# razorheadfx/aether_primitives

Hardware: AMD Instinct MI355X
Metric: GSamples/s cf32 (FFT-2048 + 64-tap FIR chain) (higher is better)
Workload: dtype f32; 1 GPU; C3: 64-tap FIR via overlap-save (FFT-2048) on 16 Mi cf32 samples per step (one fused kernel launch), device-resident, rotating over 6 stream pairs = 1536 MiB; fft_len=2048, ntaps=64, hop=1984, queues_per_gpu=2, parallelism=1 independent stream(s), one per GPU, no collective

## Files before the change

### aether_primitives_amd/csrc/aeth_fft_core.h

```cpp
#pragma once

#include <hip/hip_runtime.h>

#ifndef AETH_LDS_DB_LIMIT
#define AETH_LDS_DB_LIMIT (36 * 1024)
#endif

namespace aeth {
namespace fftk {

typedef float cf __attribute__((ext_vector_type(2)));

__device__ __forceinline__ cf mk(float a, float b) { cf r = {a, b}; return r; }

__device__ __forceinline__ cf cadd(cf a, cf b)
{
    cf d; asm("v_pk_add_f32 %0, %1, %2" : "=v"(d) : "v"(a), "v"(b)); return d;
}
__device__ __forceinline__ cf csub(cf a, cf b)
{
    cf d; asm("v_pk_add_f32 %0, %1, %2 neg_lo:[0,1] neg_hi:[0,1]" : "=v"(d) : "v"(a), "v"(b)); return d;
}
__device__ __forceinline__ cf cadd_mjb(cf a, cf b)
{
    cf d; asm("v_pk_add_f32 %0, %1, %2 op_sel:[0,1] op_sel_hi:[1,0] neg_lo:[0,0] neg_hi:[0,1]" : "=v"(d) : "v"(a), "v"(b));
    return d;
}
__device__ __forceinline__ cf cadd_pjb(cf a, cf b)
{
    cf d; asm("v_pk_add_f32 %0, %1, %2 op_sel:[0,1] op_sel_hi:[1,0] neg_lo:[0,1] neg_hi:[0,0]" : "=v"(d) : "v"(a), "v"(b));
    return d;
}
template <int S> __device__ __forceinline__ cf cadd_rot(cf a, cf b) { return S < 0 ? cadd_mjb(a, b) : cadd_pjb(a, b); }
template <int S> __device__ __forceinline__ cf csub_rot(cf a, cf b) { return S < 0 ? cadd_pjb(a, b) : cadd_mjb(a, b); }

// ... 147 lines not shown
        dft4_inplace<S, false>(o0, o1, o2, o3);
        u[0] = cadd(e0, o0);        u[4] = csub(e0, o0);
        bfly_w8<S, 1>(e1, o1, hh, u[1], u[5]);
        u[2] = cadd_rot<S>(e2, o2); u[6] = csub_rot<S>(e2, o2);
        bfly_w8<S, 3>(e3, o3, hh, u[3], u[7]);
    }
};

template <int S> struct Bfly<16, S> {
    static __device__ __forceinline__ void run(cf (&u)[16])
    {
        const cf hh = mk(kSqrtHalf, kSqrtHalf);
        const cf w1 = mk(kCosPi8, -kSinPi8), w3 = mk(kSinPi8, -kCosPi8), w9 = mk(-kCosPi8, kSinPi8);
        dft4_inplace<S, false>(u[0], u[4], u[8],  u[12]);
        dft4_inplace<S, false>(u[1], u[5], u[9],  u[13]);
        dft4_inplace<S, false>(u[2], u[6], u[10], u[14]);
        dft4_inplace<S, false>(u[3], u[7], u[11], u[15]);
        cf c0[4] = {u[0], u[1], u[2], u[3]};
        cf c1[4] = {u[4], ctw_k<S>(u[5], w1), cmul_w8<S, 1>(u[6], hh), ctw_k<S>(u[7], w3)};
        cf c2[4] = {u[8], cmul_w8<S, 1>(u[9], hh), u[10], cmul_w8<S, 3>(u[11], hh)};
        cf c3[4] = {u[12], ctw_k<S>(u[13], w3), cmul_w8<S, 3>(u[14], hh), ctw_k<S>(u[15], w9)};
        dft4_inplace<S, false>(c0[0], c0[1], c0[2], c0[3]);
        dft4_inplace<S, false>(c1[0], c1[1], c1[2], c1[3]);
        dft4_inplace<S, true>(c2[0], c2[1], c2[2], c2[3]);
        dft4_inplace<S, false>(c3[0], c3[1], c3[2], c3[3]);
#pragma unroll
        for (int kq = 0; kq < 4; kq++) {
            u[0 + 4 * kq] = c0[kq];
            u[1 + 4 * kq] = c1[kq];
            u[2 + 4 * kq] = c2[kq];
            u[3 + 4 * kq] = c3[kq];
        }
    }
};

constexpr double kPiD = 3.14159265358979323846264338327950288;
constexpr double c_sin_taylor(double x)
{
    double term = x, sum = x;
    for (int k = 1; k < 14; k++) { term *= -x * x / ((2 * k) * (2 * k + 1)); sum += term; }
    return sum;
}
constexpr double c_sin(double x)
{
    while (x > kPiD) x -= 2 * kPiD;
    while (x < -kPiD) x += 2 * kPiD;
    if (x > kPiD / 2) x = kPiD - x;
    if (x < -kPiD / 2) x = -kPiD - x;
    return c_sin_taylor(x);
}
constexpr double c_cos(double x) { return c_sin(x + kPiD / 2); }

template <int S> struct Bfly<3, S> {
    static __device__ __forceinline__ void run(cf (&u)[3])
    {
        constexpr float s60 = (float)c_sin(kPiD / 3);
        const cf t1 = cadd(u[1], u[2]), t2 = csub(u[1], u[2]);
        const cf y0 = cadd(u[0], t1);
        const cf h = cadd(y0, cscale_k(t1, mk(-1.5f, -1.5f)));
        const cf jt = cscale_k(t2, mk(s60, s60));
        u[0] = y0;
        u[1] = cadd_rot<S>(h, jt);
        u[2] = csub_rot<S>(h, jt);
    }
};

// ... 227 lines not shown
        }
    }
}

template <class C>
__device__ __forceinline__ void load_twiddles_lane(cf (&tw)[C::TW], const cf *__restrict__ twL, int tid)
{
    if constexpr (C::NPASS > 1) lane_tw_pass<C, 1>(tw, twL, tid, false);
    if constexpr (C::NPASS > 2) lane_tw_pass<C, 2>(tw, twL, tid, false);
    if constexpr (C::NPASS > 3) lane_tw_pass<C, 3>(tw, twL, tid, false);
}

template <class C>
__global__ void build_lane_twiddles(const cf *__restrict__ twN, cf *__restrict__ twL)
{
    const int tid = threadIdx.x;
    if (tid >= C::T) return;
    cf tw[C::TW];
    load_twiddles<C>(tw, twN, tid);
    if constexpr (C::NPASS > 1) lane_tw_pass<C, 1>(tw, twL, tid, true);
    if constexpr (C::NPASS > 2) lane_tw_pass<C, 2>(tw, twL, tid, true);
    if constexpr (C::NPASS > 3) lane_tw_pass<C, 3>(tw, twL, tid, true);
}

template <int XP> __device__ __forceinline__ void wg_barrier()
{
    if constexpr (XP & 16) {
        asm volatile("s_waitcnt lgkmcnt(0)" ::: "memory");
        __builtin_amdgcn_s_barrier();
        asm volatile("" ::: "memory");
    } else __syncthreads();
}

template <class C, int PASS, int S, int PAR, int XP = 0>
__device__ __forceinline__ void run_pass(cf (&w)[C::P], const cf (&tw)[C::TW], cf *__restrict__ lds, int tid)
{
    constexpr int R = C::radix(PASS), B = C::P / R, p = C::pbefore(PASS);
    constexpr bool last = (PASS == C::NPASS - 1);
    constexpr bool NOLDS = (XP & 4) != 0;
    cf *img = lds;
    if constexpr (!last && !NOLDS) {
        if constexpr (C::DB) img = lds + (((PAR + PASS) & 1) ? C::LDS_ELEMS : 0);
        else if constexpr (XP & 2) __builtin_amdgcn_fence(__ATOMIC_RELEASE, "workgroup");
        else wg_barrier<XP>();
    }
#pragma unroll
    for (int b = 0; b < B; b++) {
        cf u[R];
#pragma unroll
        for (int r = 0; r < R; r++) u[r] = w[b + r * B];
        if constexpr (p > 1) {
#pragma unroll
            for (int r = 1; r < R; r++) u[r] = ctw<S>(u[r], tw[C::twoff(PASS) + b * (R - 1) + (r - 1)]);
        }
        Bfly<R, S>::run(u);
        if constexpr (last || NOLDS) {
#pragma unroll
            for (int r = 0; r < R; r++) w[b + r * B] = u[r];
        } else {
            const int i = tid + b * C::T;
            const int k = i % p;
            const int j = (i - k) * R + k;
#pragma unroll
            for (int r = 0; r < R; r++) img[pidx<XP>(j + r * p)] = u[r];
        }
    }
    if constexpr (!last && !NOLDS) {
        if constexpr (XP & 1) __builtin_amdgcn_s_setprio(1);
        if constexpr (XP & 2) __builtin_amdgcn_fence(__ATOMIC_RELEASE, "workgroup");
        else wg_barrier<XP>();
#pragma unroll
        for (int m = 0; m < C::P; m++) w[m] = img[pidx<XP>(tid + m * C::T)];
        if constexpr (XP & 1) __builtin_amdgcn_s_setprio(0);
    }
}

template <class C, int S, int PAR = 0, int XP = 0>
__device__ __forceinline__ void fft_in_regs(cf (&w)[C::P], const cf (&tw)[C::TW], cf *__restrict__ lds, int tid)
{
    run_pass<C, 0, S, PAR, XP>(w, tw, lds, tid);
    if constexpr (C::NPASS > 1) run_pass<C, 1, S, PAR, XP>(w, tw, lds, tid);
    if constexpr (C::NPASS > 2) run_pass<C, 2, S, PAR, XP>(w, tw, lds, tid);
    if constexpr (C::NPASS > 3) run_pass<C, 3, S, PAR, XP>(w, tw, lds, tid);
}
template <class C> constexpr int fft_next_par(int par) { return (par + C::NPASS - 1) & 1; }

template <int N> struct CfgFor;
template <> struct CfgFor<2>    { using type = Cfg<2, 2, 2>; };
template <> struct CfgFor<4>    { using type = Cfg<4, 4, 4>; };
template <> struct CfgFor<8>    { using type = Cfg<8, 8, 8>; };
template <> struct CfgFor<16>   { using type = Cfg<16, 16, 16>; };
template <> struct CfgFor<32>   { using type = Cfg<32, 8, 8, 4>; };
template <> struct CfgFor<64>   { using type = Cfg<64, 8, 8, 8>; };
template <> struct CfgFor<128>  { using type = Cfg<128, 16, 16, 8>; };
template <> struct CfgFor<256>  { using type = Cfg<256, 16, 16, 16>; };
template <> struct CfgFor<512>  { using type = Cfg<512, 8, 8, 8, 8>; };
template <> struct CfgFor<1024> { using type = Cfg<1024, 16, 16, 16, 4>; };
template <> struct CfgFor<2048> { using type = Cfg<2048, 16, 16, 16, 8>; };
template <> struct CfgFor<4096> { using type = Cfg<4096, 16, 16, 16, 16>; };
template <> struct CfgFor<8192> { using type = Cfg<8192, 16, 16, 16, 8, 4>; };

#define AETH_POW2_SWITCH(len, BODY, DEFAULT)                                            \
    switch (len) {                                                                     \
    case 2: BODY(2); case 4: BODY(4); case 8: BODY(8); case 16: BODY(16);              \
    case 32: BODY(32); case 64: BODY(64); case 128: BODY(128); case 256: BODY(256);    \
    case 512: BODY(512); case 1024: BODY(1024); case 2048: BODY(2048);                 \
    case 4096: BODY(4096);                                                             \
    default: DEFAULT;                                                                  \
    }

#define AETH_POW2_SWITCH_XL(len, BODY, DEFAULT)                                         \
    switch (len) {                                                                     \
    case 2: BODY(2); case 4: BODY(4); case 8: BODY(8); case 16: BODY(16);              \
    case 32: BODY(32); case 64: BODY(64); case 128: BODY(128); case 256: BODY(256);    \
    case 512: BODY(512); case 1024: BODY(1024); case 2048: BODY(2048);                 \
    case 4096: BODY(4096); case 8192: BODY(8192);                                      \
// ... 6 lines not shown
```

### aether_primitives_amd/csrc/aeth_fir.hip

```cpp
#include "aeth_internal.h"
#include "aeth_fft_core.h"
#include "aeth_fft_plan.h"
#include "aeth_fir_kernel.h"
#include "aeth_host.h"

#include <cstdlib>
#include <memory>
#include <new>
#include <type_traits>
#include <vector>

using namespace aeth::fftk;


using namespace aeth::firk;

namespace {

constexpr bool fused_store_len(size_t n) { return 1024 <= n && n <= 4096; }

template <class C, bool SCALED, int MINW, bool CHIRP, int VAR, bool ONLY_NT = false>
int fmi_go(bool nt, int grid, hipStream_t stream, const FmiArgs &b)
{
    if (ONLY_NT || nt) hipLaunchKernelGGL((fmi_kernel<C, SCALED, MINW, true, CHIRP, VAR>), dim3(grid), dim3(C::WG), 0, stream, b);
// ... 34 lines not shown
                constexpr int DV = VAR | V_DEMOD | decltype(dmv)::value;
                if constexpr (kLab8) {
                    if (lab8_four) return fmi_go<C, SCALED, 4, false, DV, true>(nt, grid, stream, b);
                }
                return fmi_go<C, SCALED, 1, false, DV>(nt, grid, stream, b);
            };
            if (b.bps == 1) return demod(std::integral_constant<int, V_DM_BPSK>());
            if (b.demod_sep) return demod(std::integral_constant<int, 0>());
            return demod(std::integral_constant<int, V_DM_QGEN>());
        }
    }
    if constexpr (kStoreVariants && !SCALED) {
        if (b.dec.d > 1) {
            constexpr int DV = (VAR & ~V_XOR) | V_DECIM;
            return fmi_go<C, false, 2, false, DV>(nt, grid, stream, b);
        }
    }
    if constexpr (!(kStoreVariants && !SCALED)) {
        if (b.levels || b.parts)
            return aeth::set_error(AETH_E_UNSUPPORTED, "fused FFT*H*IFFT: no level-storing / peak-finding build of length %d", C::N);
    }
    if constexpr (kStoreVariants && !SCALED) {
        if (b.levels || b.parts) {
            const bool cnt = aeth::streams_past_cache((size_t)a.n * (b.levels ? 12 : 8));
            if (b.parts) return fmi_go<C, false, 2, false, VAR | V_PEAK>(cnt, grid, stream, b);
            if (b.level_kind == AETH_LEVEL_NORM) return fmi_go<C, false, 2, false, VAR | V_LEVEL>(cnt, grid, stream, b);
            if (b.level_kind == AETH_LEVEL_DB) return fmi_go<C, false, 2, false, VAR | V_LEVEL | V_LV_DB>(cnt, grid, stream, b);
            return fmi_go<C, false, 2, false, VAR | V_LEVEL | V_LV_POWER_DB>(cnt, grid, stream, b);
        }
    }
    if constexpr (C::F == 1 && !SCALED && C::NPASS == 3) {
        const int sp = aeth::tuning_int("AETH_FIR_SPREAD", -1);
        const bool chained = ctx->overlap && !ctx->stream_shared && ctx->last_chained;
        if (nt && (sp < 0 ? !chained : sp != 0)) return fmi_go<C, false, 1, false, VAR | V_SPREAD, true>(nt, grid, stream, b);
    }
    return fmi_go<C, SCALED, 1, false, VAR>(nt, grid, stream, b);
}

int dispatch_fmi(aeth_ctx *ctx, size_t fft_len, const FmiArgs &a, hipStream_t stream = nullptr)
{
    if (!stream) stream = aeth::ctx_stream(ctx);
    aeth::DeviceGuard dev_guard(ctx->device);
    const bool scaled = a.chirp != nullptr || !(a.s_fwd == 1.0f && a.s_bwd == 1.0f);
#if AETH_LAB
    if (fft_len == 2048 && a.bits && !a.chirp && aeth::lab_int("AETH_DEMOD_P8", 0)) {
        FmiArgs b8 = a;
        b8.twL = nullptr;
        using C8 = Cfg<2048, 8, 8, 8, 8, 4>;
        return scaled ? launch_fmi<C8, true>(ctx, b8, stream) : launch_fmi<C8, false>(ctx, b8, stream);
    }
#endif
#define AETH_BODY(NN)                                                            \
    return scaled ? launch_fmi<typename CfgFor<NN>::type, true>(ctx, a, stream)  \
                  : launch_fmi<typename CfgFor<NN>::type, false>(ctx, a, stream)
    AETH_POW2_SWITCH(fft_len, AETH_BODY, return aeth::set_error(AETH_E_UNSUPPORTED, "fused FFT*H*IFFT: length %zu", fft_len))
#undef AETH_BODY
}

bool is_pow2(size_t n) { return n && (n & (n - 1)) == 0; }

bool touch_bytes(const void *a, size_t na, const void *b, size_t nb)
{
    if (!a || !b || !na || !nb) return false;
    const uintptr_t a0 = (uintptr_t)a, a1 = a0 + na, b0 = (uintptr_t)b, b1 = b0 + nb;
    return a0 < b1 && b0 < a1;
}
bool touch(const aeth_cf32 *a, size_t na, const aeth_cf32 *b, size_t nb)
// ... 397 lines not shown
```

### aether_primitives_amd/csrc/aeth_fir_kernel.h

```cpp
#pragma once

#include "aeth_internal.h"
#include "aeth_fft_core.h"
#include "aeth_levels.h"

namespace aeth {
namespace firk {

using namespace aeth::fftk;

struct __attribute__((aligned(16))) PeakPart {
    double q;
    unsigned e;
    unsigned nnan;
};
static_assert(sizeof(PeakPart) == 16, "one 16-byte store per wave and block");
constexpr unsigned kPeakNone = 0x7fffffffu;

struct FmiArgs {
    const cf *in;
    cf *out;
    const cf *hist;
    const cf *Hf;
    const cf *twN;
// ... 2 lines not shown
    long long nblocks;
    int hop, ov, nhist;
    float s_fwd, s_bwd;
    const cf *chirp = nullptr;
    int frame_n = 0;
    int conj = 0;
    aeth::FastDiv dec = {1, 0, 0, 0};
    long long n_out = 0;
    unsigned char *bits = nullptr;
    cf tab[4] = {};
    int bps = 0, demod_compat = 0;
    int demod_sep = 0;
    float *levels = nullptr;
    int level_kind = 0;
    PeakPart *parts = nullptr;
};

enum : int {
    V_PEEL  = 1,
    V_TOUCH = 2,
    V_PRIO  = 4,
    V_TOUCH3 = 8,
    V_DECIM = 512,
    V_UNROLL2 = 4096,
    V_XOR = 2048,
    V_XCD = 8192,
    V_SPREAD = 16384,
    V_DEMOD = 1024,
    V_DM_BPSK = 1 << 16, V_DM_QGEN = 1 << 17,
    V_LEVEL = 1 << 19,
    V_LV_DB = 1 << 20, V_LV_POWER_DB = 1 << 21,
    V_PEAK = 1 << 22,
    V_DMA = 1 << 18,
    V_NOLOAD = 16,
    V_NOSTORE = 32,
    V_CENSUS = 256,
    V_NOLDS = 128,
    V_NOBAR = 64,
};

constexpr int V_PRODUCT_MASK = V_PRIO | V_XOR | V_SPREAD | V_DECIM | V_DEMOD | V_DM_BPSK | V_DM_QGEN | V_LEVEL | V_LV_DB |
                               V_LV_POWER_DB | V_PEAK;
#ifndef AETH_FIR_LAB
#define AETH_FIR_LAB 0
#endif

#ifndef AETH_FIR_LOAD_AUX
#define AETH_FIR_LOAD_AUX 2
#endif
#ifndef AETH_FIR_STORE_AUX
#define AETH_FIR_STORE_AUX 18
#endif

typedef unsigned int u32x2 __attribute__((ext_vector_type(2)));


__device__ __forceinline__ cf as_cf(u32x2 v) { return __builtin_bit_cast(cf, v); }
__device__ __forceinline__ u32x2 as_u32x2(cf v) { return __builtin_bit_cast(u32x2, v); }

template <class C, bool NT>
__device__ __forceinline__ void load_window(cf (&x)[C::P], const FmiArgs &a, long long blk, int tid)
{
    const long long win0 = blk * a.hop - a.ov;
    if (blk >= a.nblocks) {
#pragma unroll
        for (int m = 0; m < C::P; m++) x[m] = mk(0.f, 0.f);
        return;
    }
    if constexpr (C::F == 1) {
        if (win0 >= 0) {
            long long left = a.n - win0;
            int bytes = (int)(left < a.frame_n ? left : a.frame_n) * 8;
            auto rs = __builtin_amdgcn_make_buffer_rsrc(const_cast<cf *>(a.in + win0), 0, bytes, 0x00020000);
#pragma unroll
            for (int m = 0; m < C::P; m++)
// ... 3 lines not shown
    }
    if constexpr (C::F > 1) {
        const long long first = (blk - (long long)(threadIdx.x / C::T)) * a.hop - a.ov;
        const long long last_end = first + (long long)(C::F - 1) * a.hop + C::N;
        if (a.frame_n == C::N && first >= 0 && last_end <= a.n && blk - (long long)(threadIdx.x / C::T) + C::F <= a.nblocks) {
#pragma unroll
            for (int m = 0; m < C::P; m++) {
                const cf v = a.in[win0 + tid + m * C::T];
                x[m] = (tid + m * C::T >= a.ov - a.nhist) ? v : mk(0.f, 0.f);
            }
            return;
        }
        if (a.frame_n < C::N && a.ov == 0 && blk - (long long)(threadIdx.x / C::T) + C::F <= a.nblocks) {
#pragma unroll
            for (int m = 0; m < C::P; m++) {
                const int e = tid + m * C::T;
                x[m] = e < a.frame_n ? a.in[win0 + e] : mk(0.f, 0.f);
            }
            return;
        }
    }
#pragma unroll
    for (int m = 0; m < C::P; m++) {
        const long long gi = win0 + tid + m * C::T;
        cf v = mk(0.f, 0.f);
        if (tid + m * C::T >= a.ov - a.nhist && tid + m * C::T < a.frame_n) {
            if (gi >= 0) { if (gi < a.n) v = a.in[gi]; }
            else if (a.hist && gi >= -(long long)a.nhist) v = a.hist[a.nhist + gi];
        }
        x[m] = v;
    }
}

template <class C, bool NT>
__device__ __forceinline__ void load_window_srd(cf (&x)[C::P], const FmiArgs &a, long long blk, int tid)
{
    const bool active = blk < a.nblocks;
    const long long win0 = active ? blk * a.hop - a.ov : 0;
    long long left = a.n - win0;
    const int bytes = active ? (int)(left < a.frame_n ? left : a.frame_n) * 8 : 0;
    auto rs = __builtin_amdgcn_make_buffer_rsrc(const_cast<cf *>(a.in + win0), 0, bytes, 0x00020000);
#pragma unroll
    for (int m = 0; m < C::P; m++)
        x[m] = as_cf(__builtin_amdgcn_raw_buffer_load_b64(rs, (tid + m * C::T) * 8, 0, NT ? AETH_FIR_LOAD_AUX : 0));
}

template <class C, bool NT, int M0, int M1>
__device__ __forceinline__ void load_window_srd_part(cf (&x)[C::P], const FmiArgs &a, long long blk, int tid)
{
    const bool active = blk < a.nblocks;
    const long long win0 = active ? blk * a.hop - a.ov : 0;
    long long left = a.n - win0;
    const int bytes = active ? (int)(left < a.frame_n ? left : a.frame_n) * 8 : 0;
    auto rs = __builtin_amdgcn_make_buffer_rsrc(const_cast<cf *>(a.in + win0), 0, bytes, 0x00020000);
#pragma unroll
    for (int m = M0; m < M1; m++)
        x[m] = as_cf(__builtin_amdgcn_raw_buffer_load_b64(rs, (tid + m * C::T) * 8, 0, NT ? AETH_FIR_LOAD_AUX : 0));
    __builtin_amdgcn_sched_barrier(0);
}

typedef __attribute__((address_space(3))) void *lds_vptr_t;
template <bool NT>
__device__ __forceinline__ void dma_piece(__amdgpu_buffer_rsrc_t rs, cf *dst, int voff, int soff)
{
#if __HIP_DEVICE_COMPILE__
    __builtin_amdgcn_raw_ptr_buffer_load_lds(rs, (lds_vptr_t)dst, 16, voff, soff, 0, NT ? AETH_FIR_LOAD_AUX : 0);
#endif
}
template <class C, bool NT, int J0, int J1>
__device__ __forceinline__ void dma_window_part(cf *land, const FmiArgs &a, long long blk, int tid)
{
    static_assert(C::T == 128 && C::P == 16, "landing image: two waves, sixteen rows of 1 KiB");
    const bool active = blk < a.nblocks;
    const long long win0 = active ? blk * a.hop - a.ov : 0;
    long long left = a.n - win0;
    const int bytes = active ? (int)(left < a.frame_n ? left : a.frame_n) * 8 : 0;
    auto rs = __builtin_amdgcn_make_buffer_rsrc(const_cast<cf *>(a.in + win0), 0, bytes, 0x00020000);
    const int wv = tid >> 6, l = tid & 63;
    const int voff = (l >> 5) * 1024 + wv * 512 + (l & 31) * 16;
#pragma unroll
    for (int j = J0; j < J1; j++) dma_piece<NT>(rs, land + wv * 1024 + j * 128, voff, j * 2048);
    __builtin_amdgcn_sched_barrier(0);
}
template <class C> __device__ __forceinline__ int land_slot(int tid, int m) { return (tid >> 6) * 1024 + (m >> 1) * 128 + (m & 1) * 64 + (tid & 63); }

template <class C>
__device__ __forceinline__ unsigned touch_window(const FmiArgs &a, long long blk, int tid)
{
    const bool active = blk < a.nblocks;
    const long long win0 = active ? blk * a.hop - a.ov : 0;
// ... 150 lines not shown
#pragma unroll
        for (int m = 0; m < C::P; m++) {
            const int e = tid + m * C::T;
            const unsigned o = o0 + (unsigned)(e - a.ov);
            const unsigned q = aeth::fdiv(o, a.dec);
            const bool keep = e >= a.ov && q * a.dec.d == o && (long long)o < a.n;
            const int off = keep ? (int)(q - q0) * 8 : 0x7ffffff0;
            cf v = SCALED ? cscale_k(w[m], ss) : w[m];
            __builtin_amdgcn_raw_buffer_store_b64(as_u32x2(v), rs, off, 0, NT ? AETH_FIR_STORE_AUX : 0);
        }
    } else if constexpr (C::F == 1) {
        long long left = a.n - base;
        int bytes = (int)(left < a.frame_n ? left : a.frame_n) * 8;
        if constexpr (!CHECK) { if (blk >= a.nblocks) bytes = 0; }
        auto rs = __builtin_amdgcn_make_buffer_rsrc(a.out + base, 0, bytes, 0x00020000);
        const cf ss = mk(a.s_bwd, a.s_bwd);
#pragma unroll
        for (int m = 0; m < C::P; m++) {
            const int e = tid + m * C::T;
            const int off = (e >= a.ov) ? e * 8 : 0x7ffffff0;
            cf v = SCALED ? cscale_k(w[m], ss) : w[m];
            __builtin_amdgcn_raw_buffer_store_b64(as_u32x2(v), rs, off, 0, NT ? AETH_FIR_STORE_AUX : 0);
        }
    } else {
#pragma unroll
        for (int m = 0; m < C::P; m++) {
            const int e = tid + m * C::T;
            const long long o = base + e;
            if (e >= a.ov && o < a.n && e < a.frame_n) a.out[o] = SCALED ? cscale(w[m], a.s_bwd) : w[m];
        }
    }
}

template <class C, bool NT, int VAR>
__device__ __forceinline__ void transform_block_spread(cf (&w)[C::P], cf (&nx)[C::P], const cf (&tw)[C::TW], const cf (&H)[C::P],
                                                       cf *__restrict__ lds, const FmiArgs &a, long long gn, int tid)
{
    static_assert(C::NPASS == 3 && C::P % 4 == 0, "spread loads: three passes");
    constexpr int XP = ((VAR & V_PRIO) ? 1 : 0) | ((VAR & V_XOR) ? 8 : 0);
    constexpr int Q = C::P / 4;
    load_window_srd_part<C, NT, 0, Q>(nx, a, gn, tid);
    run_pass<C, 0, +1, 0, XP>(w, tw, lds, tid);
    load_window_srd_part<C, NT, Q, 2 * Q>(nx, a, gn, tid);
    run_pass<C, 1, +1, 0, XP>(w, tw, lds, tid);
    load_window_srd_part<C, NT, 2 * Q, 3 * Q>(nx, a, gn, tid);
    run_pass<C, 2, +1, 0, XP>(w, tw, lds, tid);
#pragma unroll
    for (int m = 0; m < C::P; m++) w[m] = cmul(w[m], H[m]);
    load_window_srd_part<C, NT, 3 * Q, 4 * Q>(nx, a, gn, tid);
    fft_in_regs<C, -1, fft_next_par<C>(0), XP>(w, tw, lds, tid);
}

template <class C, bool SCALED, bool BLU, int VAR>
__device__ __forceinline__ void transform_block(cf (&w)[C::P], const cf (&tw)[C::TW], const cf (&H)[C::P],
                                                cf *__restrict__ lds, const FmiArgs &a, int tid)
{
    constexpr int XP = ((VAR & V_PRIO) ? 1 : 0) | ((VAR & V_NOBAR) ? 2 : 0) | ((VAR & V_NOLDS) ? 4 : 0) | ((VAR & V_XOR) ? 8 : 0);
    if constexpr (BLU) {
        auto cr = __builtin_amdgcn_make_buffer_rsrc(const_cast<cf *>(a.chirp), 0, a.frame_n * 8, 0x00020000);
#pragma unroll
        for (int m = 0; m < C::P; m++) {
            const cf ch = as_cf(__builtin_amdgcn_raw_buffer_load_b64(cr, (tid + m * C::T) * 8, 0, 0));
            cf v = w[m];
            if (a.conj) v.y = -v.y;
            w[m] = cmul(v, ch);
        }
    }
    fft_in_regs<C, +1, 0, XP>(w, tw, lds, tid);
    if constexpr (SCALED) {
        const cf ss = mk(a.s_fwd, a.s_fwd);
#pragma unroll
        for (int m = 0; m < C::P; m++) w[m] = cscale_k(w[m], ss);
    }
#pragma unroll
    for (int m = 0; m < C::P; m++) w[m] = cmul(w[m], H[m]);
    fft_in_regs<C, -1, fft_next_par<C>(0), XP>(w, tw, lds, tid);
    if constexpr (BLU) {
        auto cr = __builtin_amdgcn_make_buffer_rsrc(const_cast<cf *>(a.chirp), 0, a.frame_n * 8, 0x00020000);
#pragma unroll
        for (int m = 0; m < C::P; m++) {
            const cf ch = as_cf(__builtin_amdgcn_raw_buffer_load_b64(cr, (tid + m * C::T) * 8, 0, 0));
            cf v = cmul(w[m], ch);
            if (a.conj) v.y = -v.y;
            w[m] = v;
        }
    }
}

template <class C, bool SCALED, int MINW, bool NT, bool BLU, int VAR = 0>
__global__ __launch_bounds__(C::WG, MINW) void fmi_kernel(FmiArgs a)
{
    static_assert(AETH_FIR_LAB || (VAR & ~V_PRODUCT_MASK) == 0, "lab-only kernel variant in a product build");
    __shared__ cf lds_all[C::LDS_TOTAL];
    const int tid = (C::F == 1) ? (int)threadIdx.x : (int)(threadIdx.x % C::T);
    const int fl = (C::F == 1) ? 0 : (int)(threadIdx.x / C::T);
    cf *lds = lds_all + fl * C::LDS_FRAME;

    if constexpr (VAR & V_CENSUS) {
        if ((threadIdx.x & 63) == 0) {
            unsigned *cb = reinterpret_cast<unsigned *>(const_cast<cf *>(a.chirp));
            const unsigned slot = blockIdx.x * (C::WG / 64) + threadIdx.x / 64;
            cb[2 * slot] = __builtin_amdgcn_s_getreg((4) | (0 << 6) | (31 << 11));
            cb[2 * slot + 1] = __builtin_amdgcn_s_getreg((20) | (0 << 6) | (31 << 11));
        }
    }
    const long long ngroups = (a.nblocks + C::F - 1) / C::F;
    constexpr bool PEEL = (VAR & V_PEEL) && C::F == 1 && !BLU;
    constexpr bool TOUCH = (VAR & V_TOUCH) && C::F == 1 && !BLU;
    constexpr int TOUCH_AHEAD = (VAR & V_TOUCH3) ? 3 : 2;
    cf nx[C::P], tw[C::TW], H[C::P];
    constexpr int DM = (VAR & V_DM_BPSK) ? DM_BPSK : (VAR & V_DM_QGEN) ? DM_QGEN : DM_QSEP;
    static_assert(!(VAR & (V_DM_BPSK | V_DM_QGEN)) || (VAR & V_DEMOD), "decision mode without V_DEMOD");
    [[maybe_unused]] DemodK dk;
    if constexpr (VAR & V_DEMOD) dk = demod_consts<DM>(a);
    constexpr int LK = (VAR & V_LV_DB) ? AETH_LEVEL_DB : (VAR & V_LV_POWER_DB) ? AETH_LEVEL_POWER_DB : AETH_LEVEL_NORM;
    static_assert(!(VAR & (V_LV_DB | V_LV_POWER_DB)) || (VAR & V_LEVEL), "level kind without V_LEVEL");
    static_assert(!(VAR & (V_LEVEL | V_PEAK)) || (C::F == 1 && !BLU && !(VAR & (V_PEEL | V_UNROLL2 | V_DEMOD | V_DECIM))),
                  "level store / peak search: the plain loop of one-block workgroups");
    unsigned bid = blockIdx.x;
    if constexpr ((VAR & V_XCD) != 0) {
        if ((gridDim.x & 7u) == 0) bid = (blockIdx.x & 7u) * (gridDim.x >> 3) + (blockIdx.x >> 3);
    }
    long long g0 = bid;
    unsigned tprev = 0;

    if constexpr (PEEL) {
        cf w[C::P];
        if (bid == 0) load_window<C, NT>(w, a, 0, tid);
        else load_window_srd<C, NT>(w, a, g0, tid);
        if (a.twL) load_twiddles_lane<C>(tw, a.twL, tid);
        else load_twiddles<C>(tw, a.twN, tid);
#pragma unroll
        for (int m = 0; m < C::P; m++) H[m] = a.Hf[tid + m * C::T];
        load_window_srd<C, NT>(nx, a, g0 + gridDim.x, tid);
        if constexpr (TOUCH) {
#pragma unroll
            for (int k = 2; k <= TOUCH_AHEAD; k++) tprev |= touch_window<C>(a, g0 + (long long)k * gridDim.x, tid);
        }
        if (tid < a.ov - a.nhist) w[0] = mk(0.f, 0.f);
        transform_block<C, SCALED, BLU, VAR>(w, tw, H, lds, a, tid);
        if constexpr (VAR & V_DEMOD) demod_block<C, SCALED, NT, DM>(w, a, dk, g0, tid);
        else store_block<C, SCALED, NT, false, (VAR & V_DECIM) != 0>(w, a, g0, tid);
        g0 += gridDim.x;
    } else {
        load_window<C, NT>(nx, a, (long long)bid * C::F + fl, tid);
        if (a.twL) load_twiddles_lane<C>(tw, a.twL, tid);
        else load_twiddles<C>(tw, a.twN, tid);
#pragma unroll
        for (int m = 0; m < C::P; m++) H[m] = a.Hf[tid + m * C::T];
        __builtin_amdgcn_s_waitcnt(0x0F70);
    }
    if constexpr ((VAR & V_UNROLL2) && C::F == 1 && !BLU && !(VAR & (V_DEMOD | V_DECIM | V_TOUCH | V_NOLOAD | V_NOSTORE))) {
        cf wb[C::P];
        auto one = [&](cf (&cur)[C::P], cf (&nxt)[C::P], long long g) {
            if (tid < a.ov - a.nhist) cur[0] = mk(0.f, 0.f);
            load_window_srd<C, NT>(nxt, a, g + gridDim.x, tid);
            transform_block<C, SCALED, BLU, VAR>(cur, tw, H, lds, a, tid);
            store_block<C, SCALED, NT, false, false>(cur, a, g, tid);
        };
#pragma unroll 1
        for (long long g = g0; g < ngroups; g += 2 * (long long)gridDim.x) {
            one(nx, wb, g);
            one(wb, nx, g + gridDim.x);
        }
        return;
    }
#pragma unroll 1
    for (long long g = g0; g < ngroups; g += gridDim.x) {
        const long long blk = g * C::F + fl;
        cf w[C::P];
#pragma unroll
        for (int m = 0; m < C::P; m++) w[m] = nx[m];
        if constexpr (C::F == 1) { if (tid < a.ov - a.nhist) w[0] = mk(0.f, 0.f); }
        const long long gn = g + gridDim.x;
        if constexpr (VAR & V_NOLOAD) {
#pragma unroll
            for (int m = 0; m < C::P; m++) asm volatile("" : "+v"(nx[m]));
        } else if constexpr (C::F == 1 && (VAR & V_SPREAD) && !SCALED && !BLU) {
        } else if constexpr (C::F == 1) {
            load_window_srd<C, NT>(nx, a, gn, tid);
        } else {
            if (gn < ngroups) load_window<C, NT>(nx, a, gn * C::F + fl, tid);
        }
        if constexpr (TOUCH) {
            asm volatile("" ::"v"(tprev));
            tprev = touch_window<C>(a, g + (long long)TOUCH_AHEAD * gridDim.x, tid);
        }
        if constexpr (C::F == 1 && (VAR & V_SPREAD) && !SCALED && !BLU) transform_block_spread<C, NT, VAR>(w, nx, tw, H, lds, a, gn, tid);
        else transform_block<C, SCALED, BLU, VAR>(w, tw, H, lds, a, tid);
        if constexpr (VAR & V_NOSTORE) {
#pragma unroll
            for (int m = 0; m < C::P; m++) asm volatile("" ::"v"(w[m]));
        } else if constexpr (VAR & V_DEMOD) demod_block<C, SCALED, NT, DM>(w, a, dk, blk, tid);
        else if constexpr (VAR & V_LEVEL) level_block<C, SCALED, NT, LK>(w, a, blk, tid);
        else if constexpr (VAR & V_PEAK) peak_block<C, SCALED, NT>(w, a, blk, tid);
        else store_block<C, SCALED, NT, true, (VAR & V_DECIM) != 0>(w, a, blk, tid);
    }
    if constexpr (TOUCH) asm volatile("" ::"v"(tprev));
}

template <class C> struct OneImg : C { static constexpr bool DB = false; static constexpr int LDS_TOTAL = C::LDS_ELEMS; };

template <class C0, bool NT, int VAR>
__global__ __launch_bounds__(C0::WG, 1) void fmi_dma_kernel(FmiArgs a)
{
    using C = OneImg<C0>;
    static_assert(C::F == 1 && C::T == 128 && C::P == 16 && C::NPASS == 3, "landing image layout: N = 2048");
    static_assert(AETH_FIR_LAB || (VAR & ~V_PRODUCT_MASK) == 0, "lab-only kernel variant in a product build");
    __shared__ __attribute__((aligned(1024))) cf lds_all[C::N + C::LDS_TOTAL];
    cf *land = lds_all, *lds = lds_all + C::N;
    const int tid = (int)threadIdx.x;
    constexpr int XP = ((VAR & V_PRIO) ? 1 : 0) | ((VAR & V_XOR) ? 8 : 0) | 16;
    cf tw[C::TW], H[C::P];
    const long long g0 = blockIdx.x;
    if (blockIdx.x == 0) {
        cf w0[C::P];
        load_window<C, NT>(w0, a, 0, tid);
#pragma unroll
        for (int m = 0; m < C::P; m++) land[land_slot<C>(tid, m)] = w0[m];
// ... 41 lines not shown
```

Measured before the change: 350.7 GSamples/s.

## Overlap output stores with last FFT pass butterflies in fused FIR kernel

Result: no change. 350.6 GSamples/s (-0.0%).

```diff
diff --git a/aether_primitives_amd/csrc/aeth_fft_core.h b/aether_primitives_amd/csrc/aeth_fft_core.h
--- a/aether_primitives_amd/csrc/aeth_fft_core.h
+++ b/aether_primitives_amd/csrc/aeth_fft_core.h
@@ -1,6 +1,8 @@
 #pragma once
 
 #include <hip/hip_runtime.h>
+
+#include <type_traits>
 
 #ifndef AETH_LDS_DB_LIMIT
 #define AETH_LDS_DB_LIMIT (36 * 1024)
@@ -214,6 +216,17 @@
             u[3 + 4 * kq] = c3[kq];
         }
     }
+    template <int Q> static __device__ __forceinline__ void row(cf (&u)[16]) { dft4_inplace<S, false>(u[Q], u[Q + 4], u[Q + 8], u[Q + 12]); }
+    template <int KP> static __device__ __forceinline__ void col(const cf (&u)[16], cf (&c)[4])
+    {
+        const cf hh = mk(kSqrtHalf, kSqrtHalf);
+        const cf w1 = mk(kCosPi8, -kSinPi8), w3 = mk(kSinPi8, -kCosPi8), w9 = mk(-kCosPi8, kSinPi8);
+        if constexpr (KP == 0) { c[0] = u[0]; c[1] = u[1]; c[2] = u[2]; c[3] = u[3]; }
+        if constexpr (KP == 1) { c[0] = u[4]; c[1] = ctw_k<S>(u[5], w1); c[2] = cmul_w8<S, 1>(u[6], hh); c[3] = ctw_k<S>(u[7], w3); }
+        if constexpr (KP == 2) { c[0] = u[8]; c[1] = cmul_w8<S, 1>(u[9], hh); c[2] = u[10]; c[3] = cmul_w8<S, 3>(u[11], hh); }
+        if constexpr (KP == 3) { c[0] = u[12]; c[1] = ctw_k<S>(u[13], w3); c[2] = cmul_w8<S, 3>(u[14], hh); c[3] = ctw_k<S>(u[15], w9); }
+        dft4_inplace<S, KP == 2>(c[0], c[1], c[2], c[3]);
+    }
 };
 
 constexpr double kPiD = 3.14159265358979323846264338327950288;
@@ -507,9 +520,107 @@
     } else __syncthreads();
 }
 
-template <class C, int PASS, int S, int PAR, int XP = 0>
-__device__ __forceinline__ void run_pass(cf (&w)[C::P], const cf (&tw)[C::TW], cf *__restrict__ lds, int tid)
-{
+struct NoEmit { __device__ __forceinline__ void operator()(int) const {} };
+
+template <class C, int PASS> constexpr int first_use_slot(int i)
+{
+    return C::radix(PASS) == 16 ? (i >> 2) + 4 * (i & 3)
+                                : (i >> 3) + 4 * (i & 3) + 2 * ((i >> 2) & 1);
+}
+
+template <class C, int PASS, int S, int PAR, int XP, class Emit>
+__device__ __forceinline__ void run_pass_ov(cf (&w)[C::P], const cf (&tw)[C::TW], cf *__restrict__ lds, int tid, Emit emit)
+{
+    constexpr int R = C::radix(PASS), B = C::P / R, p = C::pbefore(PASS);
+    constexpr bool last = (PASS == C::NPASS - 1);
+    constexpr bool WCOL = (XP & 32) != 0, RORD = (XP & 64) != 0;
+    constexpr bool STEP = RORD && PASS > 0;
+    static_assert(C::P == 16 && C::DB && !(XP & (2 | 4)), "overlapped exchange: 16 points per lane, two LDS images, barriers on");
+    static_assert((R == 16 && B == 1) || (R == 8 && B == 2 && last), "overlapped exchange: radix 16, or radix 8 as the last pass");
+    cf *img = lds + (((PAR + PASS) & 1) ? C::LDS_ELEMS : 0);
+    constexpr int t0 = C::twoff(PASS);
+    if constexpr (R == 16) {
+        using BF = Bfly<16, S>;
+#define AETH_OV_ROW(Q)                                                                                   \
+        if constexpr (p > 1) {                                                                           \
+            if constexpr (Q > 0) w[Q] = ctw<S>(w[Q], tw[t0 + Q - 1]);                                    \
+            w[Q + 4] = ctw<S>(w[Q + 4], tw[t0 + Q + 3]);                                                 \
+            w[Q + 8] = ctw<S>(w[Q + 8], tw[t0 + Q + 7]);                                                 \
+            w[Q + 12] = ctw<S>(w[Q + 12], tw[t0 + Q + 11]);                                              \
+        }                                                                                                \
+        BF::template row<Q>(w);                                                                          \
+        if constexpr (STEP) __builtin_amdgcn_sched_barrier(0);
+        AETH_OV_ROW(0) AETH_OV_ROW(1) AETH_OV_ROW(2) AETH_OV_ROW(3)
+#undef AETH_OV_ROW
+        const int k = tid % p;
+        const int j = (tid - k) * R + k;
+        cf c[4][4];
+#define AETH_OV_COL(KP)                                                                                  \
+        BF::template col<KP>(w, c[KP]);                                                                  \
+        if constexpr (!last && WCOL) {                                                                   \
+            _Pragma("unroll") for (int kq = 0; kq < 4; kq++) img[pidx<XP>(j + (KP + 4 * kq) * p)] = c[KP][kq]; \
+            __builtin_amdgcn_sched_barrier(0);                                                           \
+        }
+        AETH_OV_COL(0) AETH_OV_COL(1) AETH_OV_COL(2) AETH_OV_COL(3)
+#undef AETH_OV_COL
+        if constexpr (last) {
+#pragma unroll
+            for (int kp = 0; kp < 4; kp++) {
+#pragma unroll
+                for (int kq = 0; kq < 4; kq++) w[kp + 4 * kq] = c[kp][kq];
+            }
+            emit(0);
+        } else if constexpr (!WCOL) {
+#pragma unroll
+            for (int r = 0; r < R; r++) img[pidx<XP>(j + r * p)] = c[r & 3][r >> 2];
+        }
+    } else {
+        const cf hh = mk(kSqrtHalf, kSqrtHalf);
+#pragma unroll
+        for (int b = 0; b < B; b++) {
+            cf u[8];
+#pragma unroll
+            for (int r = 0; r < 8; r++) u[r] = w[b + r * B];
+#pragma unroll
+            for (int h = 0; h < 2; h++) {
+                if constexpr (p > 1) {
+#pragma unroll
+                    for (int r = h; r < 8; r += 2)
+                        if (r > 0) u[r] = ctw<S>(u[r], tw[t0 + b * (R - 1) + (r - 1)]);
+                }
+                dft4_inplace<S, false>(u[h], u[h + 2], u[h + 4], u[h + 6]);
+                if constexpr (STEP) __builtin_amdgcn_sched_barrier(0);
+            }
+            w[b + 0 * B] = cadd(u[0], u[1]);        w[b + 4 * B] = csub(u[0], u[1]);
+            bfly_w8<S, 1>(u[2], u[3], hh, w[b + 1 * B], w[b + 5 * B]);
+            w[b + 2 * B] = cadd_rot<S>(u[4], u[5]); w[b + 6 * B] = csub_rot<S>(u[4], u[5]);
+            bfly_w8<S, 3>(u[6], u[7], hh, w[b + 3 * B], w[b + 7 * B]);
+            emit(b);
+            if constexpr (!std::is_same<Emit, NoEmit>::value) __builtin_amdgcn_sched_barrier(0);
+        }
+    }
+    if constexpr (!last) {
+        if constexpr (XP & 1) __builtin_amdgcn_s_setprio(1);
+        wg_barrier<XP>();
+        if constexpr (RORD) {
+#pragma unroll
+            for (int i = 0; i < C::P; i++) {
+                const int m = first_use_slot<C, PASS + 1>(i);
+                w[m] = img[pidx<XP>(tid + m * C::T)];
+                if ((i & 3) == 3) __builtin_amdgcn_sched_barrier(0);
+            }
+        } else {
+#pragma unroll
+            for (int m = 0; m < C::P; m++) w[m] = img[pidx<XP>(tid + m * C::T)];
+        }
+        if constexpr (XP & 1) __builtin_amdgcn_s_setprio(0);
+    }
+}
+
+template <class C, int PASS, int S, int PAR, int XP = 0, class Emit = NoEmit>
+__device__ __forceinline__ void run_pass(cf (&w)[C::P], const cf (&tw)[C::TW], cf *__restrict__ lds, int tid, Emit emit = Emit())
+{
+    if constexpr ((XP & (32 | 64)) != 0 || !std::is_same<Emit, NoEmit>::value) return run_pass_ov<C, PASS, S, PAR, XP, Emit>(w, tw, lds, tid, emit);
     constexpr int R = C::radix(PASS), B = C::P / R, p = C::pbefore(PASS);
     constexpr bool last = (PASS == C::NPASS - 1);
     constexpr bool NOLDS = (XP & 4) != 0;
@@ -550,13 +661,13 @@
     }
 }
 
-template <class C, int S, int PAR = 0, int XP = 0>
-__device__ __forceinline__ void fft_in_regs(cf (&w)[C::P], const cf (&tw)[C::TW], cf *__restrict__ lds, int tid)
-{
-    run_pass<C, 0, S, PAR, XP>(w, tw, lds, tid);
-    if constexpr (C::NPASS > 1) run_pass<C, 1, S, PAR, XP>(w, tw, lds, tid);
-    if constexpr (C::NPASS > 2) run_pass<C, 2, S, PAR, XP>(w, tw, lds, tid);
-    if constexpr (C::NPASS > 3) run_pass<C, 3, S, PAR, XP>(w, tw, lds, tid);
+template <class C, int S, int PAR = 0, int XP = 0, class Emit = NoEmit>
+__device__ __forceinline__ void fft_in_regs(cf (&w)[C::P], const cf (&tw)[C::TW], cf *__restrict__ lds, int tid, Emit emit = Emit())
+{
+    run_pass<C, 0, S, PAR, XP, Emit>(w, tw, lds, tid, emit);
+    if constexpr (C::NPASS > 1) run_pass<C, 1, S, PAR, XP, Emit>(w, tw, lds, tid, emit);
+    if constexpr (C::NPASS > 2) run_pass<C, 2, S, PAR, XP, Emit>(w, tw, lds, tid, emit);
+    if constexpr (C::NPASS > 3) run_pass<C, 3, S, PAR, XP, Emit>(w, tw, lds, tid, emit);
 }
 template <class C> constexpr int fft_next_par(int par) { return (par + C::NPASS - 1) & 1; }
 
diff --git a/aether_primitives_amd/csrc/aeth_fir.hip b/aether_primitives_amd/csrc/aeth_fir.hip
--- a/aether_primitives_amd/csrc/aeth_fir.hip
+++ b/aether_primitives_amd/csrc/aeth_fir.hip
@@ -90,7 +90,8 @@
     if constexpr (C::F == 1 && !SCALED && C::NPASS == 3) {
         const int sp = aeth::tuning_int("AETH_FIR_SPREAD", -1);
         const bool chained = ctx->overlap && !ctx->stream_shared && ctx->last_chained;
-        if (nt && (sp < 0 ? !chained : sp != 0)) return fmi_go<C, false, 1, false, VAR | V_SPREAD, true>(nt, grid, stream, b);
+        constexpr int LONE = VAR | V_SPREAD | ((C::N == 2048 && C::P == 16) ? V_OVS : 0);
+        if (nt && (sp < 0 ? !chained : sp != 0)) return fmi_go<C, false, 1, false, LONE, true>(nt, grid, stream, b);
     }
     return fmi_go<C, SCALED, 1, false, VAR>(nt, grid, stream, b);
 }
diff --git a/aether_primitives_amd/csrc/aeth_fir_kernel.h b/aether_primitives_amd/csrc/aeth_fir_kernel.h
--- a/aether_primitives_amd/csrc/aeth_fir_kernel.h
+++ b/aether_primitives_amd/csrc/aeth_fir_kernel.h
@@ -58,6 +58,10 @@
     V_LV_DB = 1 << 20, V_LV_POWER_DB = 1 << 21,
     V_PEAK = 1 << 22,
     V_DMA = 1 << 18,
+    V_OVW = 1 << 23,
+    V_OVR = 1 << 24,
+    V_OVS = 1 << 25,
+    V_HALO = 1 << 26,
     V_NOLOAD = 16,
     V_NOSTORE = 32,
     V_CENSUS = 256,
@@ -66,7 +70,12 @@
 };
 
 constexpr int V_PRODUCT_MASK = V_PRIO | V_XOR | V_SPREAD | V_DECIM | V_DEMOD | V_DM_BPSK | V_DM_QGEN | V_LEVEL | V_LV_DB |
-                               V_LV_POWER_DB | V_PEAK;
+                               V_LV_POWER_DB | V_PEAK | V_OVS;
+template <int VAR> constexpr int xp_of()
+{
+    return ((VAR & V_PRIO) ? 1 : 0) | ((VAR & V_NOBAR) ? 2 : 0) | ((VAR & V_NOLDS) ? 4 : 0) | ((VAR & V_XOR) ? 8 : 0) |
+           ((VAR & V_OVW) ? 32 : 0) | ((VAR & V_OVR) ? 64 : 0);
+}
 #ifndef AETH_FIR_LAB
 #define AETH_FIR_LAB 0
 #endif
@@ -136,7 +145,7 @@
     }
 }
 
-template <class C, bool NT>
+template <class C, bool NT, bool HALO = false>
 __device__ __forceinline__ void load_window_srd(cf (&x)[C::P], const FmiArgs &a, long long blk, int tid)
 {
     const bool active = blk < a.nblocks;
@@ -144,12 +153,23 @@
     long long left = a.n - win0;
     const int bytes = active ? (int)(left < a.frame_n ? left : a.frame_n) * 8 : 0;
     auto rs = __builtin_amdgcn_make_buffer_rsrc(const_cast<cf *>(a.in + win0), 0, bytes, 0x00020000);
+    if constexpr (HALO && NT && C::T == 128) {
+        const bool wave0 = __builtin_amdgcn_readfirstlane(tid) < 64;
+        if (wave0) x[0] = as_cf(__builtin_amdgcn_raw_buffer_load_b64(rs, tid * 8, 0, 0));
+        else x[0] = as_cf(__builtin_amdgcn_raw_buffer_load_b64(rs, tid * 8, 0, AETH_FIR_LOAD_AUX));
+#pragma unroll
+        for (int m = 1; m < C::P - 1; m++)
+            x[m] = as_cf(__builtin_amdgcn_raw_buffer_load_b64(rs, (tid + m * C::T) * 8, 0, AETH_FIR_LOAD_AUX));
+        if (wave0) x[C::P - 1] = as_cf(__builtin_amdgcn_raw_buffer_load_b64(rs, (tid + (C::P - 1) * C::T) * 8, 0, AETH_FIR_LOAD_AUX));
+        else x[C::P - 1] = as_cf(__builtin_amdgcn_raw_buffer_load_b64(rs, (tid + (C::P - 1) * C::T) * 8, 0, 0));
+        return;
+    }
 #pragma unroll
     for (int m = 0; m < C::P; m++)
         x[m] = as_cf(__builtin_amdgcn_raw_buffer_load_b64(rs, (tid + m * C::T) * 8, 0, NT ? AETH_FIR_LOAD_AUX : 0));
 }
 
-template <class C, bool NT, int M0, int M1>
+template <class C, bool NT, int M0, int M1, bool HALO = false>
 __device__ __forceinline__ void load_window_srd_part(cf (&x)[C::P], const FmiArgs &a, long long blk, int tid)
 {
     const bool active = blk < a.nblocks;
@@ -158,8 +178,17 @@
     const int bytes = active ? (int)(left < a.frame_n ? left : a.frame_n) * 8 : 0;
     auto rs = __builtin_amdgcn_make_buffer_rsrc(const_cast<cf *>(a.in + win0), 0, bytes, 0x00020000);
 #pragma unroll
-    for (int m = M0; m < M1; m++)
+    for (int m = M0; m < M1; m++) {
+        if constexpr (HALO && NT && C::T == 128) {
+            if (m == 0 || m == C::P - 1) {
+                const bool wave0 = __builtin_amdgcn_readfirstlane(tid) < 64;
+                if (wave0 == (m == 0)) x[m] = as_cf(__builtin_amdgcn_raw_buffer_load_b64(rs, (tid + m * C::T) * 8, 0, 0));
+                else x[m] = as_cf(__builtin_amdgcn_raw_buffer_load_b64(rs, (tid + m * C::T) * 8, 0, AETH_FIR_LOAD_AUX));
+                continue;
+            }
+        }
         x[m] = as_cf(__builtin_amdgcn_raw_buffer_load_b64(rs, (tid + m * C::T) * 8, 0, NT ? AETH_FIR_LOAD_AUX : 0));
+    }
     __builtin_amdgcn_sched_barrier(0);
 }
 
@@ -376,30 +405,56 @@
     }
 }
 
-template <class C, bool NT, int VAR>
+template <class C, bool NT>
+struct StoreEmit {
+    __amdgpu_buffer_rsrc_t rs;
+    const cf (&w)[C::P];
+    int tid, ov;
+    __device__ __forceinline__ StoreEmit(const cf (&w_)[C::P], const FmiArgs &a, long long blk, int tid_) : w(w_), tid(tid_), ov(a.ov)
+    {
+        static_assert(C::F == 1, "one block per workgroup");
+        const long long base = blk * a.hop - a.ov;
+        long long left = a.n - base;
+        int bytes = (int)(left < a.frame_n ? left : a.frame_n) * 8;
+        if (blk >= a.nblocks) bytes = 0;
+        rs = __builtin_amdgcn_make_buffer_rsrc(a.out + base, 0, bytes, 0x00020000);
+    }
+    __device__ __forceinline__ void operator()(int b) const
+    {
+        constexpr int R = C::radix(C::NPASS - 1), B = C::P / R;
+#pragma unroll
+        for (int r = 0; r < R; r++) {
+            const int e = tid + (b + r * B) * C::T;
+            const int off = (e >= ov) ? e * 8 : 0x7ffffff0;
+            __builtin_amdgcn_raw_buffer_store_b64(as_u32x2(w[b + r * B]), rs, off, 0, NT ? AETH_FIR_STORE_AUX : 0);
+        }
+    }
+};
+
+template <class C, bool NT, int VAR, class Emit = NoEmit>
 __device__ __forceinline__ void transform_block_spread(cf (&w)[C::P], cf (&nx)[C::P], const cf (&tw)[C::TW], const cf (&H)[C::P],
-                                                       cf *__restrict__ lds, const FmiArgs &a, long long gn, int tid)
+                                                       cf *__restrict__ lds, const FmiArgs &a, long long gn, int tid, Emit emit = Emit())
 {
     static_assert(C::NPASS == 3 && C::P % 4 == 0, "spread loads: three passes");
-    constexpr int XP = ((VAR & V_PRIO) ? 1 : 0) | ((VAR & V_XOR) ? 8 : 0);
+    constexpr int XP = xp_of<VAR & (V_PRIO | V_XOR | V_OVW | V_OVR)>();
     constexpr int Q = C::P / 4;
-    load_window_srd_part<C, NT, 0, Q>(nx, a, gn, tid);
+    load_window_srd_part<C, NT, 0, Q, (VAR & V_HALO) != 0>(nx, a, gn, tid);
     run_pass<C, 0, +1, 0, XP>(w, tw, lds, tid);
-    load_window_srd_part<C, NT, Q, 2 * Q>(nx, a, gn, tid);
+    load_window_srd_part<C, NT, Q, 2 * Q, (VAR & V_HALO) != 0>(nx, a, gn, tid);
     run_pass<C, 1, +1, 0, XP>(w, tw, lds, tid);
-    load_window_srd_part<C, NT, 2 * Q, 3 * Q>(nx, a, gn, tid);
+    load_window_srd_part<C, NT, 2 * Q, 3 * Q, (VAR & V_HALO) != 0>(nx, a, gn, tid);
     run_pass<C, 2, +1, 0, XP>(w, tw, lds, tid);
 #pragma unroll
     for (int m = 0; m < C::P; m++) w[m] = cmul(w[m], H[m]);
-    load_window_srd_part<C, NT, 3 * Q, 4 * Q>(nx, a, gn, tid);
-    fft_in_regs<C, -1, fft_next_par<C>(0), XP>(w, tw, lds, tid);
-}
-
-template <class C, bool SCALED, bool BLU, int VAR>
+    load_window_srd_part<C, NT, 3 * Q, 4 * Q, (VAR & V_HALO) != 0>(nx, a, gn, tid);
+    fft_in_regs<C, -1, fft_next_par<C>(0), XP, Emit>(w, tw, lds, tid, emit);
+}
+
+template <class C, bool SCALED, bool BLU, int VAR, class Emit = NoEmit>
 __device__ __forceinline__ void transform_block(cf (&w)[C::P], const cf (&tw)[C::TW], const cf (&H)[C::P],
-                                                cf *__restrict__ lds, const FmiArgs &a, int tid)
-{
-    constexpr int XP = ((VAR & V_PRIO) ? 1 : 0) | ((VAR & V_NOBAR) ? 2 : 0) | ((VAR & V_NOLDS) ? 4 : 0) | ((VAR & V_XOR) ? 8 : 0);
+                                                cf *__restrict__ lds, const FmiArgs &a, int tid, Emit emit = Emit())
+{
+    constexpr int XP = xp_of<VAR>();
     if constexpr (BLU) {
         auto cr = __builtin_amdgcn_make_buffer_rsrc(const_cast<cf *>(a.chirp), 0, a.frame_n * 8, 0x00020000);
 #pragma unroll
@@ -418,7 +473,7 @@
     }
 #pragma unroll
     for (int m = 0; m < C::P; m++) w[m] = cmul(w[m], H[m]);
-    fft_in_regs<C, -1, fft_next_par<C>(0), XP>(w, tw, lds, tid);
+    fft_in_regs<C, -1, fft_next_par<C>(0), XP, Emit>(w, tw, lds, tid, emit);
     if constexpr (BLU) {
         auto cr = __builtin_amdgcn_make_buffer_rsrc(const_cast<cf *>(a.chirp), 0, a.frame_n * 8, 0x00020000);
 #pragma unroll
@@ -461,6 +516,9 @@
     static_assert(!(VAR & (V_LV_DB | V_LV_POWER_DB)) || (VAR & V_LEVEL), "level kind without V_LEVEL");
     static_assert(!(VAR & (V_LEVEL | V_PEAK)) || (C::F == 1 && !BLU && !(VAR & (V_PEEL | V_UNROLL2 | V_DEMOD | V_DECIM))),
                   "level store / peak search: the plain loop of one-block workgroups");
+    static_assert(!(VAR & (V_OVW | V_OVR | V_OVS)) || (C::F == 1 && C::P == 16 && C::NPASS == 3 && !SCALED && !BLU && !(VAR & (V_PEEL | V_UNROLL2 | V_NOBAR | V_NOLDS))),
+                  "overlapped exchanges: the plain loop of the unscaled 16-point-per-lane, three-pass builds");
+    static_assert(!(VAR & V_OVS) || !(VAR & (V_DEMOD | V_DECIM | V_LEVEL | V_PEAK | V_NOSTORE)), "stores per butterfly: the plain sample store");
     unsigned bid = blockIdx.x;
     if constexpr ((VAR & V_XCD) != 0) {
         if ((gridDim.x & 7u) == 0) bid = (blockIdx.x & 7u) * (gridDim.x >> 3) + (blockIdx.x >> 3);
@@ -522,13 +580,19 @@
             for (int m = 0; m < C::P; m++) asm volatile("" : "+v"(nx[m]));
         } else if constexpr (C::F == 1 && (VAR & V_SPREAD) && !SCALED && !BLU) {
         } else if constexpr (C::F == 1) {
-            load_window_srd<C, NT>(nx, a, gn, tid);
+            load_window_srd<C, NT, (VAR & V_HALO) != 0>(nx, a, gn, tid);
         } else {
             if (gn < ngroups) load_window<C, NT>(nx, a, gn * C::F + fl, tid);
         }
         if constexpr (TOUCH) {
             asm volatile("" ::"v"(tprev));
             tprev = touch_window<C>(a, g + (long long)TOUCH_AHEAD * gridDim.x, tid);
+        }
+        if constexpr (VAR & V_OVS) {
+            const StoreEmit<C, NT> st(w, a, blk, tid);
+            if constexpr (VAR & V_SPREAD) transform_block_spread<C, NT, VAR>(w, nx, tw, H, lds, a, gn, tid, st);
+            else transform_block<C, SCALED, BLU, VAR>(w, tw, H, lds, a, tid, st);
+            continue;
         }
         if constexpr (C::F == 1 && (VAR & V_SPREAD) && !SCALED && !BLU) transform_block_spread<C, NT, VAR>(w, nx, tw, H, lds, a, gn, tid);
         else transform_block<C, SCALED, BLU, VAR>(w, tw, H, lds, a, tid);
```
